# yangtaihong59/Rethink_Acoustic_Image_Enhancement

Measured on AMD Instinct MI355X. Metric: images/sec KDLAE-T 1×512×512 fp32 at 1/2/4/8 MI355X; PSNR vs ref, higher is better.
Workload: dtype fp32; 1 GPU; KDLAE-T forward bs=16/GPU 512x512 fp32 (static=train, params=cat, BiasFree); global_batch=16, per_gpu_batch=16, H=512, W=512, parallelism=dp1 (batch-sharded, no data-path collective)

## Files before the change

### rethink_acoustic_image_enhancement_amd/csrc/kdlae_t.cpp

```cpp
#include <hip/hip_runtime.h>

#include <algorithm>
#include <cmath>
#include <cstdio>
#include <cstdlib>
#include <cstring>
#include <string>
#include <unordered_map>
#include <vector>

#include "runtime.h"

namespace kdlae {

struct BlockW {
  int C = 0, heads = 0, Ch = 0, hid = 0, hidS = 0;
  Gemm qkv, pin, pout, proj_gemm;
  size_t dwqkv = kNone, dwqkv_b = kNone, proj = kNone, proj_b = kNone, temp = kNone;
  size_t dwffn = kNone, dwffn_b = kNone;
  bool fused_gdfn = false;
  bool gdfn_split = false;
  bool fused_attn_in = false;
  bool attn_in_split = false;
  Gemm pin_g0, pin_g1;
  bool ffn_fused = false;
  bool mdta_fused = false;
  bool attn_out_dw = false;
};

}

using namespace kdlae;

struct kdlae_t_handle : HandleBase {
  kdlae_t_config cfg{};
  std::vector<BlockW> enc1, enc2, enc3, latent, dec3, dec2, dec1, refinement, refinement_out, enhance;
  SmallW patch_embed, output, output_param, output2, cen, outputen;
  Gemm down1_2, down2_3, down3_4, up4_3, up3_2, up2_1, upen, reduce3, reduce2;
  size_t zeros = kNone;
  size_t sr_fold = kNone;
  int probe_class = 0, probe_level = 0;
  std::vector<hipEvent_t> ev;
  size_t ev_used = 0;
  double probe_bytes = 0, probe_flops = 0;
  long long probe_launches = 0;
  struct ProbeRec { std::string tag; double bytes, flops; };
  std::vector<ProbeRec> probe_recs;
  std::vector<float*> taps;

  const float* P(size_t off) const { return dw.P(off); }
  const float* P3(size_t off) const { return dw.P3(off); }
};

namespace kdlae {

static int validate(const kdlae_t_config& c) {
  if (c.dual_pixel_task)
    return fail(KDLAE_ENOTIMPL, "dual_pixel_task=True: the reference forward raises NameError (out_hq undefined, KDLAE_model.py:305-321)");
  if (c.dim <= 0 || c.dim % 16)
    return fail(KDLAE_EINVAL_CONFIG, "dim must be a positive multiple of 16 on the HIP path");
  if (c.inp_channels < 1 || c.inp_channels > 4 || c.out_channels < 1 || c.out_channels > 3)
    return fail(KDLAE_EINVAL_CONFIG, "inp_channels must be 1..4 and out_channels 1..3");
  if (c.inp_channels != c.out_channels)
    return fail(KDLAE_EINVAL_CONFIG, "inp_channels must equal out_channels (hq = out + inp_img, KDLAE_model.py:321)");
  for (int i = 0; i < 4; ++i)
    if (c.num_blocks[i] < 0 || c.heads[i] <= 0) return fail(KDLAE_EINVAL_CONFIG, "bad num_blocks/heads");
  if (c.num_refinement_blocks < 0) return fail(KDLAE_EINVAL_CONFIG, "bad num_refinement_blocks");
  auto head_ok = [&](int C, int heads) {
    if (C % heads) return false;
    const int ch = C / heads;
    if (ch % 16) return false;
    return ch / 16 >= 1 && ch / 16 <= 8;
  };
  const int d = c.dim;
  const int levels[4] = {d, 2 * d, 4 * d, 8 * d};
  for (int i = 0; i < 4; ++i)
    if (!head_ok(levels[i], c.heads[i]))
      return fail(KDLAE_EINVAL_CONFIG, "channels per head must be a multiple of 16 in [16, 128] at every level");
  if (!head_ok(2 * d, c.heads[0]))
    return fail(KDLAE_EINVAL_CONFIG, "channels per head of decoder_level1/refinement must be a multiple of 16 in [16, 128]");
  if (c.ffn_expansion_factor <= 0) return fail(KDLAE_EINVAL_CONFIG, "bad ffn_expansion_factor");
  return KDLAE_OK;
}

struct Stage {
  const char* name;
  int count, C, heads, num, den;
  std::vector<BlockW> kdlae_t_handle::*blocks;
  bool packed;
  bool runs;
  int part;
};
static std::vector<Stage> stages(const kdlae_t_config& c) {
  using H = kdlae_t_handle;
  const int d = c.dim, nr = c.num_refinement_blocks;
  const int *nb = c.num_blocks, *hd = c.heads;
  const bool cat = c.params_cat != 0, sr = c.static_train != 0;
  return {
      {"encoder_level1", nb[0], d, hd[0], 1, 1, &H::enc1, true, true, 0},
      {"encoder_level2", nb[1], 2 * d, hd[1], 1, 2, &H::enc2, true, true, 0},
      {"encoder_level3", nb[2], 4 * d, hd[2], 1, 4, &H::enc3, true, true, 0},
      {"latent", nb[3], 8 * d, hd[3], 1, 8, &H::latent, true, true, 0},
      {"decoder_level3", nb[2], 4 * d, hd[2], 1, 4, &H::dec3, true, true, 0},
      {"decoder_level2", nb[1], 2 * d, hd[1], 1, 2, &H::dec2, true, true, 0},
      {"decoder_level1", nb[0], 2 * d, hd[0], 1, 1, &H::dec1, true, true, 0},
      {"refinement", nr, 2 * d, hd[0], 1, 1, &H::refinement, true, true, 0},
      {"refinement_out", nr, 2 * d, hd[0], 1, 1, &H::refinement_out, true, cat, 1},
      {"enhance", nr, d, hd[0], 2, 1, &H::enhance, sr, sr, 2},
  };
}

struct Packer {
  kdlae_t_handle* h;
  PackProgram& prog;
  int err = KDLAE_OK;

  int32_t get(const std::string& k) { return h->ps.base(k, &err); }

  template <class F>
  size_t pack(int ntiles, int kgroups, F Wf) {
    return prog.add(pack_fragments(ntiles, kgroups, Wf));
  }
  template <class F>
  void pack_gemm(Gemm& g, F Wf) {
    g.w = pack(g.ntiles, g.kgroups, Wf);
    g.w3 = prog.split(g.w, g.ntiles, g.kgroups);
  }

  template <class RowMap>
  Gemm pointwise(const std::string& name, int Cout, int Cin, int Kpad, int nstore, RowMap row_map,
                 const std::string& ln_prefix, bool conv_bias, bool prefer_single_k) {
    Gemm g;
    const int32_t W = get(name + ".weight");
    const int32_t lnw = ln_prefix.empty() ? -1 : get(ln_prefix + ".body.weight");
    const int32_t lnb = (!ln_prefix.empty() && !h->cfg.layernorm_biasfree) ? get(ln_prefix + ".body.bias") : -1;
    const int32_t cb = conv_bias ? get(name + ".bias") : -1;
    if (err) return g;
    g.ntiles = (nstore + 15) / 16;
    g.kgroups = Kpad / 16;
    g.N = nstore;
    g.K = Kpad;
    g.ksize = 1;
    g.n_true = Cout;
    g.k_true = Cin;
    pack_gemm(g, [&](int n, int k) -> PEx {
      if (n >= nstore || k >= Cin) return PEx{};
      const int src = row_map(n);
      if (src < 0) return PEx{};
      return PEx{W + src * Cin + k, lnw >= 0 ? lnw + k : -1};
    });
    if (cb >= 0 || lnb >= 0) {
      std::vector<PEx> bv((size_t)g.ntiles * 16);
      if (lnb < 0)
        for (int n = 0; n < nstore; ++n) {
          const int src = row_map(n);
          if (src >= 0) bv[n].a = cb + src;
        }
      g.bias = prog.add(bv);
      if (lnb >= 0)
        for (int n = 0; n < nstore; ++n) {
          const int src = row_map(n);
          if (src < 0) continue;
          PDot d;
          d.dst = (int64_t)g.bias + n;
          d.base = cb >= 0 ? cb + src : -1;
          d.w = W + src * Cin;
          d.v = lnb;
          d.K = Cin;
          prog.dots.push_back(d);
        }
    }
    choose_variant(g, prefer_single_k);
    return g;
  }

  Gemm conv3(const std::string& name, int Cout, int Cin, int out_mode) {
    Gemm g;
    g.out_mode = out_mode;
    const int32_t W = get(name + ".weight");
    if (err) return g;
    g.ksize = 3;
    g.cg_per_tap = Cin / 16;
    g.ntiles = (Cout + 15) / 16;
    g.kgroups = 9 * Cin / 16;
    g.N = Cout;
    g.K = 9 * Cin;
    g.n_true = Cout;
    g.k_true = 9 * Cin;
    pack_gemm(g, [&](int n, int k) -> PEx {
      if (n >= Cout) return PEx{};
      const int tap = k / Cin, c = k - tap * Cin;
      return PEx{W + (n * Cin + c) * 9 + tap, -1};
    });
// ... 465 lines not shown
    HIPCHK(launch_dwconv_gate(ga, s));
    if ((rc = probe_end(3, b.C, 4.0 * P * 3 * b.hid, 2.0 * P * 18.0 * b.hid))) return rc;
    return gemm(b.pout, h->P3(b.pout.w3), 0, View{buf(pl.fg), b.hidS}, Hh, Ww, x, 0, x.p, x.ld, 0, 0, b.C);
  }

  int block(const BlockW& b, View x, int Hh, int Ww, const View* ffn = nullptr) {
    const bool fuse_in = b.fused_attn_in && !ffn;
    bool dw_out = false;
    int rc;
    if ((rc = gram_pass(b, x, Hh, Ww, ffn != nullptr, &dw_out))) return rc;
    if ((rc = attn_out(b, x, Hh, Ww, fuse_in, dw_out))) return rc;
    if ((rc = tap(x, b.C, Hh, Ww))) return rc;
    return feed_forward(b, x, Hh, Ww, fuse_in, ffn);
  }

  size_t tap_i = 0;
  int tap(View x, int C, int Hh, int Ww) {
    const size_t i = tap_i++;
    if (i < h->taps.size() && h->taps[i]) {
      const size_t P = (size_t)B * Hh * Ww;
      HIPCHK(hipMemcpy2DAsync(h->taps[i], (size_t)C * 4, x.p, (size_t)x.ld * 4, (size_t)C * 4, P,
                              hipMemcpyDeviceToDevice, s));
    }
    return KDLAE_OK;
  }
  int stage(const std::vector<BlockW>& st, View x, int Hh, int Ww) {
    if (st.empty()) return KDLAE_OK;
    int rc = tap(x, st[0].C, Hh, Ww);
    if (rc) return rc;
    bool fused = st.size() % 2 == 0;
    for (const BlockW& b : st) fused = fused && b.ffn_fused;
    const View T{buf(pl.fpre), st[0].C};
    View cur = x;
    for (size_t i = 0; i < st.size(); ++i) {
      const BlockW& b = st[i];
      if (fused) {
        const View nxt = (i % 2 == 0) ? T : x;
        if ((rc = block(b, cur, Hh, Ww, &nxt))) return rc;
        cur = nxt;
      } else {
        if ((rc = block(b, x, Hh, Ww))) return rc;
      }
      if ((rc = tap(cur, b.C, Hh, Ww))) return rc;
    }
    return KDLAE_OK;
  }

  int small_in(const SmallW& w, const float* in, long long sb, long long sc, long long sy, long long sx, int Hh,
               int Ww, View out, int dil) {
    SmallInParams p{};
    p.in = in;
    p.sb = sb;
    p.sc = sc;
    p.sy = sy;
    p.sx = sx;
    p.Cin = w.Cin;
    p.Cout = w.Cout;
    p.dil = dil;
    p.w = h->P(w.w);
    p.bias = h->P(w.bias);
    p.out = out.p;
    p.ldo = out.ld;
    p.Bn = B;
    p.H = Hh;
    p.W = Ww;
    p.F = 1;
    p.kt = 1;
    p.st = 0;
    p.relu = 0;
    HIPCHK(launch_conv_small_in(p, s));
    return KDLAE_OK;
  }

  int small_out(const SmallW& w, View in, int Hh, int Ww, float* out, int nchw, int ldo, const float* res,
                const float* extra) {
    SmallOutParams p{};
    p.in = in.p;
    p.ld = in.ld;
    p.Cin = w.Cin;
    p.Cout = w.Cout;
    p.w = h->P(w.w);
    p.bias = h->P(w.bias);
    p.Bn = B;
    p.H = Hh;
    p.W = Ww;
    p.F = 1;
    p.ks = 3;
    p.out = out;
    p.out_nchw = nchw;
    p.ldo = ldo;
    p.res = res;
    p.extra = extra;
    HIPCHK(launch_conv_small_out(p, s));
    return KDLAE_OK;
  }

  int trunk(const float* img, int H, int W) {
    const kdlae_t_config& c = h->cfg;
    const int d = c.dim;
    int rc;
    const int H2 = H / 2, W2 = W / 2, H3 = H / 4, W3 = W / 4, H4 = H / 8, W4 = W / 8;
    float* L1 = buf(pl.catL1);
    float* L2 = buf(pl.catL2);
    float* L3 = buf(pl.catL3);
    View e1{L1 + d, 2 * d}, e2{L2 + 2 * d, 4 * d}, e3{L3 + 4 * d, 8 * d}, lat{buf(pl.lat), 8 * d};
    const long long HW = (long long)H * W;
    const int ci = c.inp_channels;
    if ((rc = small_in(h->patch_embed, img, ci * HW, HW, W, 1, H, W, e1, 1))) return rc;
    if ((rc = stage(h->enc1, e1, H, W))) return rc;
    if ((rc = gemm(h->down1_2, h->P3(h->down1_2.w3), 0, e1, H, W, e2, 1, nullptr, 0, 0, 0, -1))) return rc;
    if ((rc = stage(h->enc2, e2, H2, W2))) return rc;
    if ((rc = gemm(h->down2_3, h->P3(h->down2_3.w3), 0, e2, H2, W2, e3, 1, nullptr, 0, 0, 0, -1))) return rc;
    if ((rc = stage(h->enc3, e3, H3, W3))) return rc;
    if ((rc = gemm(h->down3_4, h->P3(h->down3_4.w3), 0, e3, H3, W3, lat, 1, nullptr, 0, 0, 0, -1))) return rc;
    if ((rc = stage(h->latent, lat, H4, W4))) return rc;
    if ((rc = gemm(h->up4_3, h->P3(h->up4_3.w3), 0, lat, H4, W4, View{L3, 8 * d}, 2, nullptr, 0, 0, 0, -1))) return rc;
    View d3{buf(pl.dec3), 4 * d};
    if ((rc = gemm(h->reduce3, h->P3(h->reduce3.w3), 0, View{L3, 8 * d}, H3, W3, d3, 0, nullptr, 0, 0, 0, -1))) return rc;
    if ((rc = stage(h->dec3, d3, H3, W3))) return rc;
    if ((rc = gemm(h->up3_2, h->P3(h->up3_2.w3), 0, d3, H3, W3, View{L2, 4 * d}, 2, nullptr, 0, 0, 0, -1))) return rc;
    View d2{buf(pl.dec2), 2 * d};
    if ((rc = gemm(h->reduce2, h->P3(h->reduce2.w3), 0, View{L2, 4 * d}, H2, W2, d2, 0, nullptr, 0, 0, 0, -1))) return rc;
    if ((rc = stage(h->dec2, d2, H2, W2))) return rc;
    if ((rc = gemm(h->up2_1, h->P3(h->up2_1.w3), 0, d2, H2, W2, View{L1, 2 * d}, 2, nullptr, 0, 0, 0, -1))) return rc;
    View d1{L1, 2 * d};
    if ((rc = stage(h->dec1, d1, H, W))) return rc;
    return stage(h->refinement, d1, H, W);
  }

  int rate_tail(int H, int W) {
    const long long HW = (long long)H * W;
    int rc;
    View ro{buf(pl.refo), 2 * h->cfg.dim};
    if ((rc = small_in(h->output_param, buf(pl.out4), 4 * HW, 1, 4LL * W, 4, H, W, ro, 2))) return rc;
    return stage(h->refinement_out, ro, H, W);
  }

  int sr_head(const float* hq, int H, int W, float* sr) {
    const int d = h->cfg.dim, co = h->cfg.out_channels;
    const long long HW = (long long)H * W;
    int rc;
    View sv{buf(pl.srs), d};
    if (h->sr_fold != kNone) {
      SrFoldParams q{};
      q.in = hq;
      q.Cin = co;
      q.w = h->P(h->sr_fold);
      q.ntiles = 4 * d / 16;
      q.out = sv.p;
      q.ldo = sv.ld;
      q.Bn = B;
      q.H = H;
      q.W = W;
      HIPCHK(launch_sr_fold(q, s));
    } else {
      View cb{buf(pl.cenb), 2 * d};
      if ((rc = small_in(h->cen, hq, co * HW, HW, W, 1, H, W, cb, 1))) return rc;
      if ((rc = gemm(h->upen, h->P3(h->upen.w3), 0, cb, H, W, sv, 2, nullptr, 0, 0, 0, -1))) return rc;
    }
    if ((rc = stage(h->enhance, sv, 2 * H, 2 * W))) return rc;
    return small_out(h->outputen, sv, 2 * H, 2 * W, sr, 1, 0, nullptr, nullptr);
  }

  int run(const float* img, const float* rate, int H, int W, float* hq, float* sr) {
    const kdlae_t_config& c = h->cfg;
    const int d = c.dim;
    int rc;
    if ((rc = trunk(img, H, W))) return rc;
    View d1{buf(pl.catL1), 2 * d};
    if (c.params_cat) {
      if ((rc = small_out(h->output, d1, H, W, buf(pl.out4), 0, 4, nullptr, rate))) return rc;
      if ((rc = rate_tail(H, W))) return rc;
      if ((rc = small_out(h->output2, View{buf(pl.refo), 2 * d}, H, W, hq, 1, 0, img, nullptr))) return rc;
    } else {
      if ((rc = small_out(h->output, d1, H, W, hq, 1, 0, img, nullptr))) return rc;
    }
    if (c.static_train) return sr_head(hq, H, W, sr);
    return KDLAE_OK;
  }

  int run_rates(const float* img, const float* rates, int is_map, int R, int H, int W, float* hq, float* sr) {
    const kdlae_t_config& c = h->cfg;
    const int d = c.dim, co = c.out_channels, Bimg = B;
    const long long HW = (long long)H * W;
    int rc;
    if ((rc = trunk(img, H, W))) return rc;
    if ((rc = small_out(h->output, View{buf(pl.catL1), 2 * d}, H, W, buf(pl.out4t), 0, 4, nullptr, nullptr))) return rc;
    HIPCHK(launch_rate_fanout(buf(pl.out4t), rates, is_map, co, Bimg, R, HW, buf(pl.out4), s));
    B = R * Bimg;
    if ((rc = rate_tail(H, W))) return rc;
    B = Bimg;
    for (int r = 0; r < R; ++r) {
      const long long row0 = (long long)r * Bimg * HW;
      if ((rc = small_out(h->output2, View{buf(pl.refo) + row0 * 2 * d, 2 * d}, H, W, hq + row0 * co, 1, 0, img, nullptr)))
        return rc;
    }
    if (!sr) return KDLAE_OK;
    B = R * Bimg;
    return sr_head(hq, H, W, sr);
  }
};

}

extern "C" {

const char* kdlae_last_error(void) { return kdlae::g_err.c_str(); }
int kdlae_abi_version(void) { return 1; }

int kdlae_t_create(const kdlae_t_config* cfg, int device, kdlae_t_handle** out) {
  if (!cfg || !out) return fail(KDLAE_ESTATE, "null argument");
  *out = nullptr;
  int rc = validate(*cfg);
  if (rc) return rc;
  auto* h = new kdlae_t_handle();
  h->cfg = *cfg;
  h->device = device;
  teacher_keys(h->cfg, h->ps.lay);
  *out = h;
  return KDLAE_OK;
}

int kdlae_t_destroy(kdlae_t_handle* h) {
  if (!h) return KDLAE_OK;
  handle_release(h);
  {
    DeviceGuard g(h->device);
    for (hipEvent_t e : h->ev) (void)hipEventDestroy(e);
  }
  delete h;
  return KDLAE_OK;
}

int kdlae_t_num_params(const kdlae_t_handle* h) { return h ? (int)h->ps.lay.size() : 0; }

int kdlae_t_param_info(const kdlae_t_handle* h, int index, const char** name, int64_t* numel) {
  return handle_param_info(h, index, name, numel);
}

int64_t kdlae_t_params_numel(const kdlae_t_handle* h) { return h ? h->ps.lay.total : -1; }

int kdlae_t_set_param(kdlae_t_handle* h, const char* name, const float* host_data, int64_t numel) {
  return handle_set_param(h, name, host_data, numel);
}

}

static int record_program(HandleBase* base, PackProgram& prog) {
  auto* h = static_cast<kdlae_t_handle*>(base);
  const kdlae_t_config& c = h->cfg;
  Packer pk{h, prog};
  h->zeros = prog.add(std::vector<PEx>(64));
  const int d = c.dim;
  h->patch_embed = pk.small("patch_embed.proj", d, c.inp_channels, false);
  h->down1_2 = pk.conv3("down1_2.body.0", d / 2, d, 1);
  h->down2_3 = pk.conv3("down2_3.body.0", d, 2 * d, 1);
  h->down3_4 = pk.conv3("down3_4.body.0", 2 * d, 4 * d, 1);
  h->up4_3 = pk.conv3("up4_3.body.0", 16 * d, 8 * d, 2);
  h->reduce3 = pk.pointwise("reduce_chan_level3", 4 * d, 8 * d, 8 * d, 4 * d, [](int n) { return n; }, "", c.bias, false);
  h->up3_2 = pk.conv3("up3_2.body.0", 8 * d, 4 * d, 2);
  h->reduce2 = pk.pointwise("reduce_chan_level2", 2 * d, 4 * d, 4 * d, 2 * d, [](int n) { return n; }, "", c.bias, false);
  h->up2_1 = pk.conv3("up2_1.body.0", 4 * d, 2 * d, 2);
  h->output = pk.small("output", c.out_channels, 2 * d, c.bias);
  h->output_param = pk.small("output_param", 2 * d, c.out_channels + 1, c.bias);
  h->output2 = pk.small("output2", c.out_channels, 2 * d, c.bias);
  if (c.static_train) {
    const int hc = 2 * d;
    if (sr_fold_supported(c.out_channels, 2 * hc / 16) && !debug_flag("no_sr_fold")) {
      PFold& f = prog.fold;
      f.U = pk.get("upen.body.0.weight");
      f.Cw = pk.get("cen.weight");
      f.Cb = c.bias ? pk.get("cen.bias") : -1;
      f.hc = hc;
      f.cin = c.out_channels;
      if (!pk.err) h->sr_fold = prog.add(std::vector<PEx>((size_t)f.floats()));
      f.dst = pk.err ? -1 : (int64_t)h->sr_fold;
    } else {
      h->cen = pk.small("cen", hc, c.out_channels, c.bias);
      h->upen = pk.conv3("upen.body.0", 2 * hc, hc, 2);
    }
    h->outputen = pk.small("outputen", c.out_channels, hc / 2, c.bias);
  }
  for (const Stage& st : stages(c))
    if (st.packed) h->*st.blocks = pk.stage(st);
  return pk.err;
}

extern "C" {

int kdlae_t_commit_params(kdlae_t_handle* h, void* stream) { return handle_commit(h, record_program, stream); }

int kdlae_t_prepare(kdlae_t_handle* h) { return handle_prepare(h, record_program); }

int kdlae_t_pack_device(kdlae_t_handle* h, const float* params, int64_t numel, void* stream) {
  return handle_pack_device(h, record_program, params, numel, stream);
}

int64_t kdlae_t_workspace_bytes(const kdlae_t_handle* h, int B, int H, int W) {
  if (!h || !h->committed) {
    fail(KDLAE_ESTATE, "workspace_bytes needs committed params");
    return -1;
  }
  if (B <= 0 || H <= 0 || W <= 0 || H % 8 || W % 8) {
    fail(KDLAE_EINVAL_SHAPE, "B, H, W must be positive with H % 8 == 0 and W % 8 == 0");
    return -1;
  }
  return (int64_t)make_plan(h, B, H, W).total;
}

int kdlae_t_forward(kdlae_t_handle* h, const float* img, const float* rate, int B, int H, int W, float* hq,
                    float* sr, void* workspace, int64_t workspace_bytes, void* stream) {
  if (!h) return fail(KDLAE_ESTATE, "null handle");
  if (!h->committed) return fail(KDLAE_ESTATE, "forward before kdlae_t_commit_params / kdlae_t_pack_device");
  if (B <= 0 || H <= 0 || W <= 0 || H % 8 || W % 8)
    return fail(KDLAE_EINVAL_SHAPE, "KDLAE_teacher needs H % 8 == 0 and W % 8 == 0 (pixel_unshuffle x3, KDLAE_model.py:187)");
  if (!img || !hq) return fail(KDLAE_ESTATE, "img and hq are required");
  if (h->cfg.params_cat && !rate) return fail(KDLAE_ESTATE, "denoise_rate is required when params=='cat'");
  if ((sr != nullptr) != (h->cfg.static_train != 0))
    return fail(KDLAE_ESTATE, "sr must be non-null iff static=='train'");
  Fwd f{h, reinterpret_cast<hipStream_t>(stream), reinterpret_cast<char*>(workspace), make_plan(h, B, H, W), B};
  if ((int64_t)f.pl.total > workspace_bytes) return fail(KDLAE_ESTATE, "workspace too small");
  DeviceGuard g(h->device);
  return f.run(img, rate, H, W, hq, sr);
}

static int check_rates(const kdlae_t_handle* h, int B, int R, int H, int W, bool with_sr) {
  if (R < 1 || R > 64) return fail(KDLAE_EINVAL_SHAPE, "a rate sweep takes 1 <= R <= 64 rates, got " + std::to_string(R));
  if (B <= 0 || H <= 0 || W <= 0 || H % 8 || W % 8)
    return fail(KDLAE_EINVAL_SHAPE, "KDLAE_teacher needs H % 8 == 0 and W % 8 == 0 (pixel_unshuffle x3, KDLAE_model.py:187)");
  if ((long long)R * B > 0x7fffffffLL / ((long long)H * W))
    return fail(KDLAE_EINVAL_SHAPE, "R * B * H * W must stay below 2^31 pixels");
  if (!h->cfg.params_cat)
    return fail(KDLAE_EINVAL_CONFIG, "a rate sweep needs params=='cat': with params=='plus' the forward never reads denoise_rate");
  if (with_sr && !h->cfg.static_train)
    return fail(KDLAE_EINVAL_CONFIG, "sr asked for, but static != 'train': the model has no sr head");
  return KDLAE_OK;
}

static bool taps_armed(const kdlae_t_handle* h) {
  return std::any_of(h->taps.begin(), h->taps.end(), [](const float* p) { return p != nullptr; });
}

int64_t kdlae_t_rates_workspace_bytes(const kdlae_t_handle* h, int B, int R, int H, int W, int with_sr) {
  if (!h) {
    fail(KDLAE_ESTATE, "null handle");
    return -1;
  }
  if (check_rates(h, B, R, H, W, with_sr != 0)) return -1;
  if (!h->committed) {
    fail(KDLAE_ESTATE, "workspace_bytes needs committed params");
    return -1;
  }
  return (int64_t)make_plan(h, {B, R * B, with_sr ? R * B : 0}, H, W, true).total;
}

int kdlae_t_forward_rates(kdlae_t_handle* h, const float* img, const float* rates, int rate_is_map, int B, int R,
                          int H, int W, float* hq, float* sr, void* workspace, int64_t workspace_bytes,
                          void* stream) {
  if (!h) return fail(KDLAE_ESTATE, "null handle");
  if (!img || !rates || !hq) return fail(KDLAE_ESTATE, "img, rates and hq are required");
  if (rate_is_map != 0 && rate_is_map != 1) return fail(KDLAE_EINVAL_CONFIG, "rate_is_map must be 0 or 1");
  int rc = check_rates(h, B, R, H, W, sr != nullptr);
  if (rc) return rc;
  if (!h->committed) return fail(KDLAE_ESTATE, "forward before kdlae_t_commit_params / kdlae_t_pack_device");
  if (taps_armed(h)) return fail(KDLAE_ESTATE, "debug taps are sized for kdlae_t_forward: disarm them before a rate sweep");
  Fwd f{h, reinterpret_cast<hipStream_t>(stream), reinterpret_cast<char*>(workspace),
        make_plan(h, {B, R * B, sr ? R * B : 0}, H, W, true), B};
  if (!workspace || (int64_t)f.pl.total > workspace_bytes) return fail(KDLAE_ESTATE, "workspace too small");
  DeviceGuard g(h->device);
  return f.run_rates(img, rates, rate_is_map, R, H, W, hq, sr);
}

int64_t kdlae_t_sr_workspace_bytes(const kdlae_t_handle* h, int B, int H, int W) {
  if (!h || !h->committed) {
    fail(KDLAE_ESTATE, "workspace_bytes needs committed params");
    return -1;
  }
  if (B <= 0 || H <= 0 || W <= 0 || H % 8 || W % 8) {
    fail(KDLAE_EINVAL_SHAPE, "B, H, W must be positive with H % 8 == 0 and W % 8 == 0");
    return -1;
  }
  if (!h->cfg.static_train) {
    fail(KDLAE_EINVAL_CONFIG, "static != 'train': the model has no sr head");
    return -1;
  }
  return (int64_t)make_plan(h, {0, 0, B}, H, W, false).total;
}

int kdlae_t_forward_sr(kdlae_t_handle* h, const float* hq, int B, int H, int W, float* sr, void* workspace,
                       int64_t workspace_bytes, void* stream) {
  if (!h) return fail(KDLAE_ESTATE, "null handle");
  if (!hq || !sr) return fail(KDLAE_ESTATE, "hq and sr are required");
  if (B <= 0 || H <= 0 || W <= 0 || H % 8 || W % 8)
    return fail(KDLAE_EINVAL_SHAPE, "KDLAE_teacher needs H % 8 == 0 and W % 8 == 0 (pixel_unshuffle x3, KDLAE_model.py:187)");
  if (!h->cfg.static_train) return fail(KDLAE_EINVAL_CONFIG, "static != 'train': the model has no sr head");
  if (!h->committed) return fail(KDLAE_ESTATE, "forward before kdlae_t_commit_params / kdlae_t_pack_device");
  if (taps_armed(h)) return fail(KDLAE_ESTATE, "debug taps are sized for kdlae_t_forward: disarm them before kdlae_t_forward_sr");
  Fwd f{h, reinterpret_cast<hipStream_t>(stream), reinterpret_cast<char*>(workspace), make_plan(h, {0, 0, B}, H, W, false), B};
  if (!workspace || (int64_t)f.pl.total > workspace_bytes) return fail(KDLAE_ESTATE, "workspace too small");
  DeviceGuard g(h->device);
  return f.sr_head(hq, H, W, sr);
}

int64_t kdlae_t_debug_sr_fold(const kdlae_t_handle* h, float* dst, int64_t capacity, void* stream) {
  if (!h || !h->committed) {
    fail(KDLAE_ESTATE, "kdlae_t_debug_sr_fold needs committed params");
    return -1;
  }
  if (h->sr_fold == kNone) return 0;
  const int64_t n = h->dw.fold.floats();
  if (!dst) return n;
  if (capacity < n) {
    fail(KDLAE_EPARAM, "kdlae_t_debug_sr_fold: dst too small");
    return -1;
  }
  DeviceGuard g(h->device);
  if (hipMemcpyAsync(dst, h->P(h->sr_fold), (size_t)n * sizeof(float), hipMemcpyDeviceToDevice,
                     reinterpret_cast<hipStream_t>(stream)) != hipSuccess) {
    fail(KDLAE_EHIP, "kdlae_t_debug_sr_fold: copy failed");
    return -1;
  }
  return n;
}

struct TapInfo { std::string name; int C, num, den; };
static std::vector<TapInfo> tap_list(const kdlae_t_handle* h) {
  std::vector<TapInfo> v;
  for (const Stage& st : stages(h->cfg)) {
    if (!st.runs || st.count <= 0) continue;
// ... 67 lines not shown
```

### rethink_acoustic_image_enhancement_amd/csrc/kernels.h

```cpp
#pragma once
#include <hip/hip_runtime.h>

#include <cstdint>
#include <stdint.h>

namespace kdlae {

constexpr int kGemmThreads = 512;
constexpr int kGemmRT = 2;
constexpr int kGemmRows = 8 * kGemmRT * 16;

struct GemmParams {
  const float* A;  int lda;
  int cg_per_tap;
  int kgroups;
  int ksize, dil;
  const float* Wp; long long w_img_stride; int ntiles;
  int N;
  const float* bias;
  float* out; int ldo;
  const float* R; int ldr;
  const float* stats;
  int ln;
  int ln_C;
// ... 55 lines not shown
  const float* res_nhwc; int ldr;
};

inline int gram_slot_floats(int Ch) { return (Ch / 16) * (Ch / 16) * 256 + 2 * Ch; }
struct GramSegs { int nseg, seg_rows; };
inline GramSegs gram_segments(int nslots, int H, int W) {
  const int nseg = W % 16 == 0 ? nslots / (W / 16) : 0;
  return {nseg, nseg ? (H + nseg - 1) / nseg : 0};
}

bool gemm_attn_in_variant(int NT, int KG, int nch);
hipError_t launch_gemm(const GemmParams& p, int NT, int KG, int wpe, int grid_x, hipStream_t s);
hipError_t launch_gemm_route(const GemmParams& p, int NT, int KG, int wpe, int grid_x, int route, hipStream_t s);
bool gemm_variant_entry(int family, int i, int* v);
bool gemm_has_variant(int NT, int KG, bool conv3, int wpe, bool resident, int out_mode);
bool gemm_has_variant2(int NT, int KG, bool conv3, int out_mode);
hipError_t launch_ln_stats(const float* x, int ld, int C, long long P, float* stats, hipStream_t s);
hipError_t launch_dwconv_gram(const GramParams& p, hipStream_t s);
hipError_t launch_dwconv_gram_route(const GramParams& p, int route, hipStream_t s);
bool gram_ring_applies(const GramParams& p);
hipError_t launch_gram_reduce(const float* partial, float* reduced, int Bn, int heads, int nslots,
                              int slot_floats, hipStream_t s);
hipError_t launch_attn_fold(const float* reduced, int slot_floats, const float* proj, const float* temp,
                            float* Mpacked, int Bn, int C, int heads, hipStream_t s);
hipError_t launch_dwconv_gate(const GateParams& p, hipStream_t s);
hipError_t launch_conv_small_in(const SmallInParams& p, hipStream_t s);
hipError_t launch_conv_small_out(const SmallOutParams& p, hipStream_t s);
hipError_t launch_maxpool2(const float* in, int ldi, float* out, int ldo, int C, long long nframes, int H, int W,
                           hipStream_t s);
hipError_t launch_rate_fanout(const float* src, const float* rates, int is_map, int ch, int B, int R, long long HW,
                              float* dst, hipStream_t s);

struct GdfnParams {
  const float* x; int ld;
  int hidS;
  const float* dw;
  const float* Wp;
  const float* bias;
  const float* R; int ldr;
  float* out; int ldo;
  int Bn, H, W;
  const float* zeros;
  int nsplit;
  int split;
};
bool gdfn_supported(int C, int hidS);
hipError_t launch_gdfn_out(const GdfnParams& p, int C, hipStream_t s);

struct AttnOutDwParams {
  const float* v; int ldv;
  const float* wdw; int ldw;
  const float* bdw;
  const float* M; long long m_img_stride;
  const float* bias;
  const float* R; int ldr;
  float* out; int ldo;
  int Bn, H, W;
  const float* zeros;
};
bool attn_out_dw_supported(int C, int H, int W, int ldv);
hipError_t launch_attn_out_dw(const AttnOutDwParams& p, int C, hipStream_t s);

struct FfnParams {
  const float* x; int ldx;
  float* out; int ldo;
  int ln;
  int hidS;
  const float* Win;
  const float* bias_in;
  const float* dw;
  const float* Wout;
  const float* bias_out;
  int Bn, H, W;
};
bool ffn_fused_supported(int C, int hidS);
hipError_t launch_ffn_fused(const FfnParams& p, int C, hipStream_t s);


struct MdtaFusedParams {
  const float* x; int ldx;
  int ln;
  const float* Wqkv;
  const float* bias;
  const float* wdw;
  const float* bdw;
  float* v_out; int ldv;
  float* partial;
  int nslots, slot_floats, nseg, seg_rows;
  int Bn, H, W;
};
bool mdta_fused_supported(int C, int heads, int H, int W, int nseg, int seg_rows);
hipError_t launch_mdta_fused(const MdtaFusedParams& p, int C, hipStream_t s);

struct PreParams {
  const uint8_t* in; int B, h, w, cin, cout, bgr;
  int gray;
  int H, W;
  float* img;
  const float* rate; float* rate_map;
};
struct PostParams {
  const float* src; int B, C, Hs, Ws;
  int h, w, scale;
  const uint8_t* lq; int cin;
  uint8_t* out;
};
hipError_t launch_preprocess_u8(const PreParams& p, hipStream_t s);
hipError_t launch_postprocess_u8(const PostParams& p, hipStream_t s);

hipError_t launch_upsample2x(const float* in, int ldi, float* out, int ldo, int C, int N, int h, int w,
                             hipStream_t s);
hipError_t launch_gap_partial(const float* in, int ld, int C, int B, long long HW, int slots, float* partial,
                              hipStream_t s);
struct HeadParams {
  const float* partial; int slots, C; float inv_hw;
  const float* wo; const float* bo; int M;
  const float* w1; const float* b1; int N1;
  const float* w2; const float* b2; int N2;
  const float* w3; const float* b3;
  float* score; int B;
};
hipError_t launch_asdqe_head(const HeadParams& p, hipStream_t s);

struct Conv3dC16Params {
  const float* in; int ldi;
  const float* wp;
  const float* bias;
  float* out; int ldo;
  int Bn, F, H, W;
  int relu;
  int kt;
};
hipError_t launch_conv3d_c16(const Conv3dC16Params& p, hipStream_t s);

struct ConvLdsParams {
  const float* in; int ldi; int cin_pad;
  const float* wp; int ntiles, kgroups;
  const float* bias;
  float* out; int ldo;
  int Bn, F, H, W;
  int kt, relu;
  const float* wp3 = nullptr;
  int out_mode = 0, nout = 0;
};
bool conv_lds_supported(int kt, int ntiles, int cin_pad);
hipError_t launch_conv_lds(const ConvLdsParams& p, hipStream_t s);

constexpr int sr_fold_ksteps(int cin) { return (25 * cin + 1 + 3) / 4; }
struct SrFoldParams {
  const float* in; int Cin;
  const float* w; int ntiles;
  float* out; int ldo;
  int Bn, H, W;
};
bool sr_fold_supported(int cin, int ntiles);
hipError_t launch_sr_fold(const SrFoldParams& p, hipStream_t s);

constexpr int kNiqeBlock = 96;
constexpr int kNiqeTaps = 7;
struct NiqeWindow {
  double w[kNiqeTaps * kNiqeTaps];
};

}
```

### rethink_acoustic_image_enhancement_amd/csrc/sr_fold.hip

```cpp
#include "kernels.h"

namespace kdlae {

namespace {

typedef float f32x4 __attribute__((ext_vector_type(4)));

constexpr int kTR = 8, kTC = 64, kPH = kTR + 4, kPW = kTC + 4;

template <int CIN, int NTW>
__global__ __launch_bounds__(256) void sr_fold_kernel(SrFoldParams p) {
  constexpr int K = 25 * CIN, KS = sr_fold_ksteps(CIN), PP = kPH * kPW;
  __shared__ float patch[CIN * PP];
  const int tid = threadIdx.x, lane = tid & 63, wave = tid >> 6;
  const int li = lane & 15, lq = lane >> 4;
  const int tx_n = (p.W + kTC - 1) / kTC, ty_n = (p.H + kTR - 1) / kTR;
  int bid = blockIdx.x;
  const int txi = bid % tx_n;
  bid /= tx_n;
  const int tyi = bid % ty_n;
  const int b = bid / ty_n;
  const int x0 = txi * kTC, y0 = tyi * kTR;
  const long long HW = (long long)p.H * p.W;
  const float* inb = p.in + (long long)b * CIN * HW;
  for (int i = tid; i < CIN * PP; i += 256) {
    const int c = i / PP, rem = i - c * PP;
    const int r = rem / kPW, x = rem - r * kPW;
    const int yy = y0 + r - 2, xx = x0 + x - 2;
    const bool ok = (unsigned)yy < (unsigned)p.H && (unsigned)xx < (unsigned)p.W;
    patch[i] = ok ? inb[c * HW + (long long)yy * p.W + xx] : 0.f;
  }
  int koff[KS];
#pragma unroll
  for (int s = 0; s < KS; ++s) {
    const int k = 4 * s + lq;
    const int kk = k < K ? k : 0;
    const int c = kk / 25, t = kk - c * 25;
    koff[s] = c * PP + (t / 5) * kPW + t % 5;
  }
  const int t0 = wave * NTW;
  float wf[NTW][KS];
  int cur = -1;
  __syncthreads();
  const int Wo = 2 * p.W;
  for (int r = 0; r < kTR; ++r) {
    const int y = y0 + r;
    if (y >= p.H) break;
    const int rc = y == 0 ? 0 : y == p.H - 1 ? 2 : 1;
    const float* wrow = p.w + ((size_t)(3 * rc) * p.ntiles + t0) * (KS * 64) + lane;
    const size_t wcls = (size_t)p.ntiles * (KS * 64);
    if (rc != cur) {
      cur = rc;
#pragma unroll
      for (int n = 0; n < NTW; ++n)
#pragma unroll
        for (int s = 0; s < KS; ++s) wf[n][s] = wrow[wcls + (n * KS + s) * 64];
    }
#pragma unroll 1
    for (int j = 0; j < kTC / 16; ++j) {
      const int xs = x0 + 16 * j;
      if (xs >= p.W) break;
      const int x = xs + li;
      const float* win = patch + r * kPW + 16 * j + li;
      float bv[KS];
#pragma unroll
      for (int s = 0; s < KS; ++s) bv[s] = 4 * s + lq == K ? 1.f : win[koff[s]];
      f32x4 acc[NTW];
#pragma unroll
      for (int n = 0; n < NTW; ++n) acc[n] = f32x4{0.f, 0.f, 0.f, 0.f};
      const bool has0 = xs == 0, has2 = xs + 16 >= p.W;
      const bool mid = !(has0 || has2) || (x >= 1 && x <= p.W - 2);
#pragma unroll
      for (int s = 0; s < KS; ++s) {
        const float v = mid ? bv[s] : 0.f;
#pragma unroll
        for (int n = 0; n < NTW; ++n) acc[n] = __builtin_amdgcn_mfma_f32_16x16x4f32(wf[n][s], v, acc[n], 0, 0, 0);
      }
      auto edge = [&](const float* we, bool on) {
#pragma unroll
        for (int s = 0; s < KS; ++s) {
          const float v = on ? bv[s] : 0.f;
#pragma unroll
          for (int n = 0; n < NTW; ++n)
            acc[n] = __builtin_amdgcn_mfma_f32_16x16x4f32(we[(n * KS + s) * 64], v, acc[n], 0, 0, 0);
        }
      };
      if (has0) edge(wrow, x == 0);
      if (has2) edge(wrow + 2 * wcls, x == p.W - 1);
      if (x >= p.W) continue;
      float* o = p.out + (((long long)b * 2 * p.H + 2 * y + (lq >> 1)) * Wo + 2 * x + (lq & 1)) * p.ldo + 4 * t0;
#pragma unroll
      for (int n = 0; n < NTW; ++n) *reinterpret_cast<f32x4*>(o + 4 * n) = acc[n];
    }
  }
}

template <int CIN>
void launch_ntw(const SrFoldParams& p, unsigned blocks, hipStream_t s) {
  switch (p.ntiles / 4) {
    case 1: hipLaunchKernelGGL((sr_fold_kernel<CIN, 1>), dim3(blocks), dim3(256), 0, s, p); break;
    case 2: hipLaunchKernelGGL((sr_fold_kernel<CIN, 2>), dim3(blocks), dim3(256), 0, s, p); break;
    case 3: hipLaunchKernelGGL((sr_fold_kernel<CIN, 3>), dim3(blocks), dim3(256), 0, s, p); break;
    default: hipLaunchKernelGGL((sr_fold_kernel<CIN, 4>), dim3(blocks), dim3(256), 0, s, p); break;
  }
}

}

bool sr_fold_supported(int cin, int ntiles) {
  return cin >= 1 && cin <= 4 && ntiles >= 4 && ntiles <= 16 && ntiles % 4 == 0;
}

hipError_t launch_sr_fold(const SrFoldParams& p, hipStream_t s) {
  if (!sr_fold_supported(p.Cin, p.ntiles) || !p.in || !p.w || !p.out || p.Bn <= 0 || p.H < 8 || p.W < 8 || p.H % 8 ||
      p.W % 8 || p.ldo < 4 * p.ntiles || p.ldo % 4 || ((uintptr_t)p.out & 15))
    return hipErrorInvalidValue;
  const long long blocks = (long long)p.Bn * ((p.H + kTR - 1) / kTR) * ((p.W + kTC - 1) / kTC);
  if (blocks > 0x7fffffffLL) return hipErrorInvalidValue;
  switch (p.Cin) {
    case 1: launch_ntw<1>(p, (unsigned)blocks, s); break;
    case 2: launch_ntw<2>(p, (unsigned)blocks, s); break;
    case 3: launch_ntw<3>(p, (unsigned)blocks, s); break;
    default: launch_ntw<4>(p, (unsigned)blocks, s); break;
  }
  return hipGetLastError();
}

}
```

Baseline: 63.29 images/s.

## Rewrite sr_fold kernel with prefetched LDS reads, batched patch load, occupancy hint

Adds a new default sr_fold kernel and keeps the old one behind a debug flag. The new kernel stages the input patch through registers in batched row loads, software-pipelines the LDS reads of the next 16-pixel group while the current MFMAs run, and precomputes the row and column trip counts. It also reloads the edge weights per tile into temporaries and sets a launch-bounds occupancy hint of 2 waves when the register budget allows. The aim is to hide LDS and global-load latency in the fused super-resolution head, at the cost of extra register pressure and an explicit waitcnt.

```diff
diff --git a/rethink_acoustic_image_enhancement_amd/csrc/kdlae_t.cpp b/rethink_acoustic_image_enhancement_amd/csrc/kdlae_t.cpp
--- a/rethink_acoustic_image_enhancement_amd/csrc/kdlae_t.cpp
+++ b/rethink_acoustic_image_enhancement_amd/csrc/kdlae_t.cpp
@@ -39,6 +39,7 @@
   Gemm down1_2, down2_3, down3_4, up4_3, up3_2, up2_1, upen, reduce3, reduce2;
   size_t zeros = kNone;
   size_t sr_fold = kNone;
+  bool sr_fold_v1 = false;
   int probe_class = 0, probe_level = 0;
   std::vector<hipEvent_t> ev;
   size_t ev_used = 0;
@@ -810,6 +811,7 @@
       q.Bn = B;
       q.H = H;
       q.W = W;
+      q.v1 = h->sr_fold_v1;
       HIPCHK(launch_sr_fold(q, s));
     } else {
       View cb{buf(pl.cenb), 2 * d};
@@ -933,6 +935,7 @@
       f.cin = c.out_channels;
       if (!pk.err) h->sr_fold = prog.add(std::vector<PEx>((size_t)f.floats()));
       f.dst = pk.err ? -1 : (int64_t)h->sr_fold;
+      h->sr_fold_v1 = debug_flag("sr_fold_v1");
     } else {
       h->cen = pk.small("cen", hc, c.out_channels, c.bias);
       h->upen = pk.conv3("upen.body.0", 2 * hc, hc, 2);
diff --git a/rethink_acoustic_image_enhancement_amd/csrc/kernels.h b/rethink_acoustic_image_enhancement_amd/csrc/kernels.h
--- a/rethink_acoustic_image_enhancement_amd/csrc/kernels.h
+++ b/rethink_acoustic_image_enhancement_amd/csrc/kernels.h
@@ -231,6 +231,7 @@
   const float* w; int ntiles;
   float* out; int ldo;
   int Bn, H, W;
+  int v1 = 0;
 };
 bool sr_fold_supported(int cin, int ntiles);
 hipError_t launch_sr_fold(const SrFoldParams& p, hipStream_t s);
diff --git a/rethink_acoustic_image_enhancement_amd/csrc/sr_fold.hip b/rethink_acoustic_image_enhancement_amd/csrc/sr_fold.hip
--- a/rethink_acoustic_image_enhancement_amd/csrc/sr_fold.hip
+++ b/rethink_acoustic_image_enhancement_amd/csrc/sr_fold.hip
@@ -9,7 +9,7 @@
 constexpr int kTR = 8, kTC = 64, kPH = kTR + 4, kPW = kTC + 4;
 
 template <int CIN, int NTW>
-__global__ __launch_bounds__(256) void sr_fold_kernel(SrFoldParams p) {
+__global__ __launch_bounds__(256) void sr_fold_v1_kernel(SrFoldParams p) {
   constexpr int K = 25 * CIN, KS = sr_fold_ksteps(CIN), PP = kPH * kPW;
   __shared__ float patch[CIN * PP];
   const int tid = threadIdx.x, lane = tid & 63, wave = tid >> 6;
@@ -95,8 +95,137 @@
   }
 }
 
+constexpr int sr_fold_waves(int ntw, int ks) { return ntw * ks + 4 * ks + 4 * ntw + 48 <= 256 ? 2 : 1; }
+
+template <int CIN, int NTW>
+__global__ __launch_bounds__(256, sr_fold_waves(NTW, sr_fold_ksteps(CIN))) void sr_fold_kernel(SrFoldParams p) {
+  constexpr int K = 25 * CIN, KS = sr_fold_ksteps(CIN), PP = kPH * kPW, ROWS = CIN * kPH;
+  __shared__ float patch[CIN * PP];
+  const int tid = threadIdx.x, lane = tid & 63, wave = tid >> 6;
+  const int li = lane & 15, lq = lane >> 4;
+  const int tx_n = (p.W + kTC - 1) / kTC, ty_n = (p.H + kTR - 1) / kTR;
+  int bid = blockIdx.x;
+  const int txi = bid % tx_n;
+  bid /= tx_n;
+  const int tyi = bid % ty_n;
+  const int b = bid / ty_n;
+  const int x0 = txi * kTC, y0 = tyi * kTR;
+  const long long HW = (long long)p.H * p.W;
+  const float* inb = p.in + (long long)b * CIN * HW;
+  {
+    const int xa = x0 - 2 + lane, xb = xa + 64;
+    const bool oka = (unsigned)xa < (unsigned)p.W, okb = lane < 4 && (unsigned)xb < (unsigned)p.W;
+    constexpr int NI = (ROWS + 3) / 4;
+    float va[NI], vb[NI];
+#pragma unroll
+    for (int i = 0; i < NI; ++i) {
+      const int rr = wave + 4 * i;
+      const int c = rr / kPH, yy = y0 + (rr - c * kPH) - 2;
+      const bool rok = rr < ROWS && (unsigned)yy < (unsigned)p.H;
+      const long long row = c * HW + (long long)yy * p.W;
+      const float a = inb[rok && oka ? row + xa : 0], bq = inb[rok && okb ? row + xb : 0];
+      va[i] = rok && oka ? a : 0.f;
+      vb[i] = rok && okb ? bq : 0.f;
+    }
+#pragma unroll
+    for (int i = 0; i < NI; ++i) {
+      const int rr = wave + 4 * i;
+      if (rr < ROWS) {
+        patch[rr * kPW + lane] = va[i];
+        if (lane < 4) patch[rr * kPW + 64 + lane] = vb[i];
+      }
+    }
+  }
+  int koff[KS];
+#pragma unroll
+  for (int s = 0; s < KS; ++s) {
+    const int k = 4 * s + lq;
+    const int kk = k < K ? k : 0;
+    const int c = kk / 25, t = kk - c * 25;
+    koff[s] = c * PP + (t / 5) * kPW + t % 5;
+  }
+  const int t0 = wave * NTW;
+  const int nrow = p.H - y0 < kTR ? p.H - y0 : kTR;
+  const int ngrp = (p.W - x0 + 15) / 16 < kTC / 16 ? (p.W - x0 + 15) / 16 : kTC / 16;
+  auto read_b = [&](int r, int j, float (&bv)[KS]) {
+    const float* win = patch + r * kPW + 16 * j + li;
+#pragma unroll
+    for (int s = 0; s < KS; ++s) bv[s] = 4 * s + lq == K ? 1.f : win[koff[s]];
+  };
+  float wf[NTW][KS];
+  int cur = -1;
+  __syncthreads();
+  float bv[KS];
+  read_b(0, 0, bv);
+  const int Wo = 2 * p.W;
+  const size_t wcls = (size_t)p.ntiles * (KS * 64);
+  for (int r = 0; r < nrow; ++r) {
+    const int y = y0 + r;
+    const int rc = y == 0 ? 0 : y == p.H - 1 ? 2 : 1;
+    const float* wrow = p.w + ((size_t)(3 * rc) * p.ntiles + t0) * (KS * 64) + lane;
+    if (rc != cur) {
+      cur = rc;
+#pragma unroll
+      for (int n = 0; n < NTW; ++n)
+#pragma unroll
+        for (int s = 0; s < KS; ++s) wf[n][s] = wrow[wcls + (n * KS + s) * 64];
+      __builtin_amdgcn_s_waitcnt(0x0f70);
+    }
+#pragma unroll 1
+    for (int j = 0; j < ngrp; ++j) {
+      const int xs = x0 + 16 * j;
+      const int x = xs + li;
+      const bool last = j + 1 == ngrp;
+      const int rn = last ? (r + 1 < nrow ? r + 1 : r) : r;
+      float bn[KS];
+      read_b(rn, last ? 0 : j + 1, bn);
+      f32x4 acc[NTW];
+#pragma unroll
+      for (int n = 0; n < NTW; ++n) acc[n] = f32x4{0.f, 0.f, 0.f, 0.f};
+      const bool has0 = xs == 0, has2 = xs + 16 >= p.W;
+      const bool mid = !(has0 || has2) || (x >= 1 && x <= p.W - 2);
+#pragma unroll
+      for (int s = 0; s < KS; ++s) {
+        const float v = mid ? bv[s] : 0.f;
+#pragma unroll
+        for (int n = 0; n < NTW; ++n) acc[n] = __builtin_amdgcn_mfma_f32_16x16x4f32(wf[n][s], v, acc[n], 0, 0, 0);
+      }
+      auto edge = [&](const float* we, bool on) {
+        asm volatile("" : "+v"(we));
+#pragma unroll
+        for (int n = 0; n < NTW; ++n) {
+          float wt[KS];
+#pragma unroll
+          for (int s = 0; s < KS; ++s) wt[s] = we[(n * KS + s) * 64];
+#pragma unroll
+          for (int s = 0; s < KS; ++s)
+            acc[n] = __builtin_amdgcn_mfma_f32_16x16x4f32(wt[s], on ? bv[s] : 0.f, acc[n], 0, 0, 0);
+        }
+      };
+      if (has0) edge(wrow, x == 0);
+      if (has2) edge(wrow + 2 * wcls, x == p.W - 1);
+      if (x < p.W) {
+        float* o = p.out + (((long long)b * 2 * p.H + 2 * y + (lq >> 1)) * Wo + 2 * x + (lq & 1)) * p.ldo + 4 * t0;
+#pragma unroll
+        for (int n = 0; n < NTW; ++n) *reinterpret_cast<f32x4*>(o + 4 * n) = acc[n];
+      }
+#pragma unroll
+      for (int s = 0; s < KS; ++s) bv[s] = bn[s];
+    }
+  }
+}
+
 template <int CIN>
 void launch_ntw(const SrFoldParams& p, unsigned blocks, hipStream_t s) {
+  if (p.v1) {
+    switch (p.ntiles / 4) {
+      case 1: hipLaunchKernelGGL((sr_fold_v1_kernel<CIN, 1>), dim3(blocks), dim3(256), 0, s, p); break;
+      case 2: hipLaunchKernelGGL((sr_fold_v1_kernel<CIN, 2>), dim3(blocks), dim3(256), 0, s, p); break;
+      case 3: hipLaunchKernelGGL((sr_fold_v1_kernel<CIN, 3>), dim3(blocks), dim3(256), 0, s, p); break;
+      default: hipLaunchKernelGGL((sr_fold_v1_kernel<CIN, 4>), dim3(blocks), dim3(256), 0, s, p); break;
+    }
+    return;
+  }
   switch (p.ntiles / 4) {
     case 1: hipLaunchKernelGGL((sr_fold_kernel<CIN, 1>), dim3(blocks), dim3(256), 0, s, p); break;
     case 2: hipLaunchKernelGGL((sr_fold_kernel<CIN, 2>), dim3(blocks), dim3(256), 0, s, p); break;
```

Result: no change. 63.65 images/s (median of 6 runs) (+0.6%).
